# APRIL-ZJU/Ctrl-VIO

Hardware: NVIDIA H100
Metric: residual+Jacobian block evaluations per second (sliding-window LM solve) (higher is better)
Workload: dtype f64

## Files before the change

ctrl-vio_b200/csrc/chol_dag.cu:

```cuda
#include <algorithm>
#include <atomic>
#include <cstdlib>

#include "chol_tiles.cuh"
#include "dmma_tiles.cuh"
#include "kernels.h"

namespace ctvio {

namespace {

constexpr unsigned long long kSentinel = 0xFFF8C0DEC0DE0001ull;
__device__ __forceinline__ unsigned smem_u32(const void* p) { return static_cast<unsigned>(__cvta_generic_to_shared(p)); }
__device__ __forceinline__ unsigned mapa_u32(unsigned addr, unsigned rank) {
  unsigned r;
  asm volatile("mapa.shared::cluster.u32 %0, %1, %2;" : "=r"(r) : "r"(addr), "r"(rank));
  return r;
}
__device__ __forceinline__ void st_cluster2(unsigned addr, double2 v) {
  asm volatile("st.shared::cluster.v2.f64 [%0], {%1, %2};" ::"r"(addr), "d"(v.x), "d"(v.y) : "memory");
}
__device__ __forceinline__ double2 ld_shared_volatile2(const double* p) {
  double2 v;
  asm volatile("ld.volatile.shared.v2.f64 {%0, %1}, [%2];" : "=d"(v.x), "=d"(v.y) : "r"(smem_u32(p)) : "memory");
  return v;
}
__device__ __forceinline__ void cluster_arrive() { asm volatile("barrier.cluster.arrive.release.aligned;" ::: "memory"); }
__device__ __forceinline__ void cluster_wait() { asm volatile("barrier.cluster.wait.acquire.aligned;" ::: "memory"); }
__device__ __forceinline__ unsigned cluster_ctarank() {
  unsigned r;
  asm volatile("mov.u32 %0, %%cluster_ctarank;" : "=r"(r));
  return r;
}
__device__ __forceinline__ unsigned cluster_nctarank() {
  unsigned r;
  asm volatile("mov.u32 %0, %%cluster_nctarank;" : "=r"(r));
  return r;
}
__device__ __forceinline__ bool is_sentinel(double v) { return static_cast<unsigned long long>(__double_as_longlong(v)) == kSentinel; }
__device__ __forceinline__ double2 ld_relaxed2(const double* p) {
  double2 v;
  asm volatile("ld.relaxed.gpu.global.v2.f64 {%0, %1}, [%2];" : "=d"(v.x), "=d"(v.y) : "l"(p) : "memory");
  return v;
}
__device__ __forceinline__ void st_relaxed2(double* p, double2 v) {
  asm volatile("st.relaxed.gpu.global.v2.f64 [%0], {%1, %2};" ::"l"(p), "d"(v.x), "d"(v.y) : "memory");
}

__device__ __forceinline__ double ld_relaxed1(const double* p) {
  double v;
  asm volatile("ld.relaxed.gpu.global.f64 %0, [%1];" : "=d"(v) : "l"(p) : "memory");
  return v;
}
__device__ __forceinline__ void st_relaxed1(double* p, double v) {
  asm volatile("st.relaxed.gpu.global.f64 [%0], %1;" ::"l"(p), "d"(v) : "memory");
}
__device__ __forceinline__ double ld_spin(const double* p) {
  double v = ld_relaxed1(p);
  while (is_sentinel(v)) v = ld_relaxed1(p);
  return v;
}
__device__ __forceinline__ double sentinel_value() { return __longlong_as_double(static_cast<long long>(kSentinel)); }

__device__ __forceinline__ void wait_flag(const int* flag, int epoch) {
  if (threadIdx.x == 0) {
    spin_until_gpu(flag, epoch);
  }
  __syncthreads();
}
__device__ __forceinline__ void wait_flags2(const int* f1, const int* f2, int epoch) {
  if (threadIdx.x == 0) {
    spin_until_gpu(f1, epoch);
  } else if (threadIdx.x == 32) {
    spin_until_gpu(f2, epoch);
  }
  __syncthreads();
}
__device__ __forceinline__ void post_flag(int* flag, int epoch) {
  __syncthreads();
  if (threadIdx.x == 0) {
    __threadfence();
    st_release_gpu(flag, epoch);
  }
}

__device__ __forceinline__ void load_tile_cg(double* dst, const double* src, int ld, int tid) {
#pragma unroll
  for (int e = tid; e < kCholNB * kCholNB / 2; e += 256) {
    const int r = e >> 5, c = (e & 31) * 2;
    *reinterpret_cast<double2*>(dst + r * kTS + c) = __ldcg(reinterpret_cast<const double2*>(src + size_t(r) * ld + c));
  }
}
__device__ __forceinline__ void store_tile_global(double* dst, int ld, const double* src, int tid) {
#pragma unroll
  for (int e = tid; e < kCholNB * kCholNB / 2; e += 256) {
    const int r = e >> 5, c = (e & 31) * 2;
    *reinterpret_cast<double2*>(dst + size_t(r) * ld + c) = *reinterpret_cast<const double2*>(src + r * kTS + c);
  }
}
__device__ __forceinline__ double sum_partials(const double* part, int n, size_t stride, double* red, int tid) {
  const int c = tid & 63, g = tid >> 6;
  double s = 0.0;
  int q = g;
  for (; q + 12 < n; q += 16) {
    double v0 = ld_relaxed1(part + size_t(q) * stride + c), v1 = ld_relaxed1(part + size_t(q + 4) * stride + c);
    double v2 = ld_relaxed1(part + size_t(q + 8) * stride + c), v3 = ld_relaxed1(part + size_t(q + 12) * stride + c);
    while (is_sentinel(v0)) v0 = ld_relaxed1(part + size_t(q) * stride + c);
    while (is_sentinel(v1)) v1 = ld_relaxed1(part + size_t(q + 4) * stride + c);
    while (is_sentinel(v2)) v2 = ld_relaxed1(part + size_t(q + 8) * stride + c);
    while (is_sentinel(v3)) v3 = ld_relaxed1(part + size_t(q + 12) * stride + c);
    s += v0; s += v1; s += v2; s += v3;
  }
  for (; q < n; q += 4) s += ld_spin(part + size_t(q) * stride + c);
  red[g * kCholNB + c] = s;
  __syncthreads();
  return tid < kCholNB ? (red[tid] + red[kCholNB + tid]) + (red[2 * kCholNB + tid] + red[3 * kCholNB + tid]) : 0.0;
}
__device__ __forceinline__ void tile_matvec(const double* Lrm, const double* v, double* out_global, int tid,
                                            double* out_shared = nullptr) {
  const int r = tid >> 2, pt = tid & 3;
  double s = 0.0;
#pragma unroll 4
  for (int c = pt; c < kCholNB; c += 4) s = fma(Lrm[r * kTS + c], v[c], s);
  s += __shfl_xor_sync(0xffffffffu, s, 1);
  s += __shfl_xor_sync(0xffffffffu, s, 2);
  if (pt == 0) {
    st_relaxed1(out_global + r, s);
    if (out_shared) out_shared[r] = s;
  }
}
}

template <unsigned MASK>
__device__ __forceinline__ void mma_masked(Frag& f, const double* pa, int sa, const double* pb, int sb, const Lane& L, int nk4) {
#pragma unroll 4
  for (int kk = 0; kk < nk4; ++kk) {
    double av[2], bv[4];
#pragma unroll
    for (int mt = 0; mt < 2; ++mt)
      if (MASK & (0xFu << (4 * mt))) av[mt] = -pa[4 * kk * sa + 8 * L.rt[mt]];
#pragma unroll
    for (int nt = 0; nt < 4; ++nt)
      if (MASK & (0x11u << nt)) bv[nt] = pb[4 * kk * sb + 8 * L.ct[nt]];
#pragma unroll
    for (int mt = 0; mt < 2; ++mt)
#pragma unroll
      for (int nt = 0; nt < 4; ++nt)
        if ((MASK >> (4 * mt + nt)) & 1u)
          asm volatile("mma.sync.aligned.m8n8k4.row.col.f64.f64.f64.f64 {%0,%1}, {%2}, {%3}, {%0,%1};"
                       : "+d"(f.c[mt][nt][0]), "+d"(f.c[mt][nt][1]) : "d"(av[mt]), "d"(bv[nt]));
  }
}
__device__ __forceinline__ void mma_dispatch(unsigned mask, Frag& f, const double* pa, int sa, const double* pb, int sb,
                                             const Lane& L, int nk4) {
  switch (mask) {
    case 0x33u: mma_masked<0x33u>(f, pa, sa, pb, sb, L, nk4); break;
    case 0xCCu: mma_masked<0xCCu>(f, pa, sa, pb, sb, L, nk4); break;
    case 0xFFu: mma_masked<0xFFu>(f, pa, sa, pb, sb, L, nk4); break;
    case 0xF1u: mma_masked<0xF1u>(f, pa, sa, pb, sb, L, nk4); break;
    case 0x73u: mma_masked<0x73u>(f, pa, sa, pb, sb, L, nk4); break;
    case 0xF0u: mma_masked<0xF0u>(f, pa, sa, pb, sb, L, nk4); break;
    default: break;
  }
}
__device__ __forceinline__ unsigned lower_mask(int warp) {
  const int wm = warp & 3, wn = warp >> 2;
  if (wn == 0) return wm == 0 ? 0xF1u : wm == 1 ? 0x73u : 0x33u;
  return wm <= 1 ? 0xF0u : wm == 2 ? 0xF1u : 0x73u;
}
__device__ __forceinline__ unsigned slab_mask(int warp, int s) {
  const int wn = warp >> 2;
  if (wn == 0) return s == 0 ? 0x33u : s == 3 ? 0xCCu : 0u;
  return s == 1 ? 0x33u : s == 2 ? 0xCCu : 0u;
}
__device__ __forceinline__ unsigned trailing_mask(int warp, int s) {
  const int wn = warp >> 2;
  if (wn == 0) return s < 3 ? 0xCCu : 0u;
  return s == 0 ? 0xFFu : s == 1 ? 0xCCu : 0u;
}

struct CholDagArgs {
  double* M;
  int npad;
  double* Lpub;
  double* Lpub_other;
  double* Spub;
  double* Spub_other;
  const double* rhs;
  double* y;
  double* yf;
  double* part;
  double* part_other;
  int* flags;
  int epoch;
  LmScalars* scal;
  const int32_t* go;
};

#ifdef CTVIO_CHOL_TIMING
__device__ unsigned long long g_dag_stamps[32 * 16];
#define DSTAMP(j, i) do { if (threadIdx.x == 0 && (j) >= 0 && (j) < 32) { unsigned long long t_; \
    asm volatile("mov.u64 %0, %%globaltimer;" : "=l"(t_)); g_dag_stamps[(j) * 16 + (i)] = t_; } } while (0)
extern "C" int ctvio_debug_fac_clk(long long* out) {
  return cudaMemcpyFromSymbol(out, g_fac_clk, sizeof(g_fac_clk)) == cudaSuccess ? 0 : -1;
}
extern "C" int ctvio_debug_dag_stamps(unsigned long long* out) {
  return cudaMemcpyFromSymbol(out, g_dag_stamps, sizeof(g_dag_stamps)) == cudaSuccess ? 0 : -1;
}
#else
#define DSTAMP(j, i)
#endif

constexpr size_t kCholDagSmem =
    (3 * size_t(kTile) + 4 * size_t(kPacket) + 16 * size_t(kTS) + 2 * size_t(kPacket) + 256 + 7 * kCholNB + 16) * sizeof(double);

__device__ __forceinline__ void tile_matvec_t(const double* St, const double* v, double* out_global, double* red, int tid,
                                              double* out_shared = nullptr) {
  const int r = tid & 63, part = tid >> 6;
  double s = 0.0;
#pragma unroll 4
  for (int c = part; c < kCholNB; c += 4) s = fma(St[c * kTS + r], v[c], s);
  red[part * kCholNB + r] = s;
  __syncthreads();
  if (tid < kCholNB) {
    const double t = (red[tid] + red[kCholNB + tid]) + (red[2 * kCholNB + tid] + red[3 * kCholNB + tid]);
    st_relaxed1(out_global + tid, t);
    if (out_shared) out_shared[tid] = t;
  }
}

__device__ __forceinline__ void trsm_pipelined(Frag& acc, const Lane& L, double* S1, double* At, double* Bp2,
                                               const double* Lpub_col, double* slab_out, const double* Ua, const double* Ub,
                                               int tid, int jstamp, const double* pk_local = nullptr, unsigned slab_remote = 0u) {
  const int warp = tid >> 5, lane = tid & 31, g = lane >> 2, q = lane & 3;
  int goff[3], soff[3];
#pragma unroll
  for (int u = 0; u < 3; ++u) {
    const int e = tid + 256 * u;
    const int r = e / 40, c = (e - r * 40) * 2;
    goff[u] = e < 640 ? r * 80 + c : -1;
    soff[u] = r * kPS + c;
  }
  const int goff3 = tid < 128 ? (tid >> 3) * 80 + 64 + (tid & 7) * 2 : -1, soff3 = (tid >> 3) * kPS + 64 + (tid & 7) * 2;
  double2 pre[3];
  auto issue = [&](int s) {
    if (pk_local) return;
    const double* src = Lpub_col + size_t(s) * kPacketG;
    if (s < 3) {
#pragma unroll
      for (int u = 0; u < 3; ++u)
        if (goff[u] >= 0) pre[u] = ld_relaxed2(src + goff[u]);
    } else if (goff3 >= 0) {
      pre[0] = ld_relaxed2(src + goff3);
    }
  };
  auto commit = [&](int s, double* Bp) {
    if (pk_local) {
      if (s < 3) {
#pragma unroll
        for (int u = 0; u < 3; ++u)
          if (goff[u] >= 0) {
            double2 v = ld_shared_volatile2(Bp + soff[u]);
            while (is_sentinel(v.x) || is_sentinel(v.y)) v = ld_shared_volatile2(Bp + soff[u]);
          }
      } else if (goff3 >= 0) {
        double2 v = ld_shared_volatile2(Bp + soff3);
        while (is_sentinel(v.x) || is_sentinel(v.y)) v = ld_shared_volatile2(Bp + soff3);
      }
      return;
    }
    const double* src = Lpub_col + size_t(s) * kPacketG;
    if (s < 3) {
#pragma unroll
      for (int u = 0; u < 3; ++u)
        if (goff[u] >= 0) {
          while (is_sentinel(pre[u].x) || is_sentinel(pre[u].y)) pre[u] = ld_relaxed2(src + goff[u]);
          *reinterpret_cast<double2*>(Bp + soff[u]) = pre[u];
        }
    } else if (goff3 >= 0) {
      while (is_sentinel(pre[0].x) || is_sentinel(pre[0].y)) pre[0] = ld_relaxed2(src + goff3);
      *reinterpret_cast<double2*>(Bp + soff3) = pre[0];
    }
  };
  issue(0);
#pragma unroll 1
  for (int s = 0; s < 4; ++s) {
    double* Bp = pk_local ? const_cast<double*>(pk_local) + s * kPacket : Bp2 + (s & 1) * kPacket;
    if (Ua) {
      if (s == 0) mma_dispatch(slab_mask(warp, 0), acc, Ua + q * kTS + g, kTS, Ub + q * kTS + g, kTS, L, kCholNB / 4);
      if (s < 3) mma_dispatch(slab_mask(warp, s + 1), acc, Ua + q * kTS + g, kTS, Ub + q * kTS + g, kTS, L, kCholNB / 4);
    }
#pragma unroll
    for (int mt = 0; mt < 2; ++mt)
#pragma unroll
      for (int nt = 0; nt < 4; ++nt) {
        const int ct = L.ct[nt];
        if ((ct >> 1) == s) {
#pragma unroll
          for (int e = 0; e < 2; ++e) At[(8 * (ct & 1) + 2 * q + e) * kTS + L.row(mt)] = acc.c[mt][nt][e];
        }
      }
    DSTAMP(16 + jstamp, 4 * s + 0);
    commit(s, Bp);
    DSTAMP(16 + jstamp, 4 * s + 1);
    if (s < 3) issue(s + 1);
    __syncthreads();
    DSTAMP(jstamp, 8 + s);
    if (s == 3) DSTAMP(jstamp, 2);
    {
      const double* pa = At + q * kTS + 8 * warp + g;
      const double* pb = Bp + q * kPS + 64 + g;
      double2 cl = make_double2(0.0, 0.0), ch = make_double2(0.0, 0.0);
#pragma unroll
      for (int kk = 0; kk < 4; ++kk) {
        const double av = pa[4 * kk * kTS];
        if (kk < 2)
          asm volatile("mma.sync.aligned.m8n8k4.row.col.f64.f64.f64.f64 {%0,%1}, {%2}, {%3}, {%0,%1};"
                       : "+d"(cl.x), "+d"(cl.y) : "d"(av), "d"(pb[4 * kk * kPS]));
        asm volatile("mma.sync.aligned.m8n8k4.row.col.f64.f64.f64.f64 {%0,%1}, {%2}, {%3}, {%0,%1};"
                     : "+d"(ch.x), "+d"(ch.y) : "d"(av), "d"(pb[4 * kk * kPS + 8]));
      }
      double* dst = S1 + (16 * s) * kTS + 8 * warp + g;
      dst[(2 * q) * kTS] = cl.x;
      dst[(2 * q + 1) * kTS] = cl.y;
      dst[(8 + 2 * q) * kTS] = ch.x;
      dst[(8 + 2 * q + 1) * kTS] = ch.y;
    }
    DSTAMP(16 + jstamp, 4 * s + 2);
    __syncthreads();
    if (slab_out) {
#pragma unroll
      for (int u = 0; u < 2; ++u) {
        const int e = tid + 256 * u, r = e >> 5, c = (e & 31) * 2;
        const double2 v = *reinterpret_cast<const double2*>(S1 + (16 * s + r) * kTS + c);
        if (slab_remote) st_cluster2(slab_remote + unsigned(((16 * s + r) * kTS + c) * sizeof(double)), v);
        st_relaxed2(slab_out + size_t(s) * 16 * 64 + r * 64 + c, v);
      }
    }
    if (s < 3)
      mma_dispatch(trailing_mask(warp, s), acc, S1 + (16 * s + q) * kTS + g, kTS, Bp + q * kPS + g, kPS, L, 4);
    DSTAMP(16 + jstamp, 4 * s + 3);
  }
}

__global__ void __launch_bounds__(256, 1) chol_dag_kernel(CholDagArgs a) {
  extern __shared__ __align__(16) unsigned char dag_smem[];
  double* D = reinterpret_cast<double*>(dag_smem);
  double* S1 = D + kTile;
  double* S2 = S1 + kTile;
  double* Pk = S2 + kTile;
  double* At = Pk + 4 * kPacket;
  double* Bp = At + 16 * kTS;
  double* L16t = Bp + 2 * kPacket;
  double* rdiag = L16t + 256;
  double* vec = rdiag + kCholNB;
  double* vec2 = vec + kCholNB;
  double* red = vec2 + kCholNB;
  double* x16 = red + 4 * kCholNB;
  __shared__ int s_bad;
  const int tid = threadIdx.x;
  const Lane L = lane_of(tid);
  const int npad = a.npad, nb = npad / kCholNB, epoch = a.epoch;
  int* tile_ready = a.flags;
  const size_t nn = size_t(nb) * nb * kCholNB;
  double* fwd_part = a.part;
  double* bwd_part = a.part + nn;
  double* xf_pub = a.part + 2 * nn;
  double* xb_pub = xf_pub + size_t(nb) * kCholNB;
  const double sv = sentinel_value();
  const bool go = !a.go || *a.go != 0;

  const int pos = blockIdx.x, nchain = 2 * nb - 1;
  const unsigned crank = cluster_ctarank(), csize = cluster_nctarank();
  const bool dsm = csize > 1;
  const bool is_diag = pos < nchain && (pos & 1) == 0;
  const bool recv_local = dsm && pos < nchain && pos > 0 && crank != 0;
  const bool send_remote = dsm && pos + 1 < nchain && crank + 1 < csize;
  if (dsm) {
    if (recv_local) {
      double* area = is_diag ? S1 : Pk;
      const int n2 = (is_diag ? kTile : 4 * kPacket) / 2;
      for (int e = tid; e < n2; e += 256) *reinterpret_cast<double2*>(area + 2 * e) = make_double2(sv, sv);
    }
    __syncthreads();
    cluster_arrive();
  }
  pdl_wait();
  pdl_launch_dependents();
  if (!go || (dsm && pos >= nb * (nb + 1) / 2)) {
    if (dsm) cluster_wait();
    return;
  }
  if (!is_diag) {
    int i, j;
    if (pos < nchain) {
      i = (pos + 1) >> 1;
      j = i - 1;
    } else {
      int t = pos - nchain;
      j = 0;
      while (t >= nb - 2 - j) { t -= nb - 2 - j; ++j; }
      i = j + 2 + t;
    }
    const bool sub = i == j + 1;
    double* slot = a.M + size_t(i) * kCholNB * npad + j * kCholNB;
    Frag acc;
    frag_load_global(acc, slot, npad, L);
    for (int k = 0; k + 1 < j; ++k) {
      wait_flags2(tile_ready + i * nb + k, tile_ready + j * nb + k, epoch);
      load_tile_cg(S1, a.M + size_t(i) * kCholNB * npad + k * kCholNB, npad, tid);
      load_tile_cg(S2, a.M + size_t(j) * kCholNB * npad + k * kCholNB, npad, tid);
      __syncthreads();
      tile_gemm_dmma<true>(S1, S2, acc, L);
      __syncthreads();
    }
    if (j >= 1) {
      const double* srcA = a.Spub + (size_t(i) * nb + (j - 1)) * 4096;
      const double* srcB = a.Spub + (size_t(j) * nb + (j - 1)) * 4096;
      const int r0 = tid >> 5, c0 = (tid & 31) * 2;
      double2 pa[2], pb[2];
      auto issue = [&](int s) {
#pragma unroll
        for (int u = 0; u < 2; ++u) {
          pa[u] = ld_relaxed2(srcA + size_t(s) * 1024 + (r0 + 8 * u) * 64 + c0);
          pb[u] = ld_relaxed2(srcB + size_t(s) * 1024 + (r0 + 8 * u) * 64 + c0);
        }
      };
      issue(0);
#pragma unroll 1
      for (int s = 0; s < 4; ++s) {
#pragma unroll
        for (int u = 0; u < 2; ++u) {
          const size_t o = size_t(s) * 1024 + (r0 + 8 * u) * 64 + c0;
          while (is_sentinel(pa[u].x) || is_sentinel(pa[u].y)) pa[u] = ld_relaxed2(srcA + o);
          while (is_sentinel(pb[u].x) || is_sentinel(pb[u].y)) pb[u] = ld_relaxed2(srcB + o);
          *reinterpret_cast<double2*>(D + (16 * s + r0 + 8 * u) * kTS + c0) = pa[u];
          *reinterpret_cast<double2*>(S2 + (16 * s + r0 + 8 * u) * kTS + c0) = pb[u];
        }
        if (s < 3) issue(s + 1);
        __syncthreads();
        mma_dispatch(0xFFu, acc, D + (16 * s + L.q) * kTS + L.g, kTS, S2 + (16 * s + L.q) * kTS + L.g, kTS, L, 4);
      }
    }
    unsigned slab_remote = 0u;
    if (dsm) {
      cluster_wait();
      if (sub && send_remote) slab_remote = mapa_u32(smem_u32(S1), crank + 1);
    }
    trsm_pipelined(acc, L, S1, At, Bp, a.Lpub + size_t(j) * 4 * kPacketG, a.Spub + (size_t(i) * nb + j) * 4096, nullptr, nullptr, tid,
                   sub ? i : -100, (sub && recv_local) ? Pk : nullptr, slab_remote);
    __syncthreads();
    store_tile_global(slot, npad, S1, tid);
    post_flag(tile_ready + i * nb + j, epoch);
    if (!sub) {
      if (tid < kCholNB) vec[tid] = ld_spin(xf_pub + j * kCholNB + tid);
      __syncthreads();
      tile_matvec_t(S1, vec, fwd_part + (size_t(i) * nb + j) * kCholNB, red, tid);
      if (tid < kCholNB) vec[tid] = ld_spin(xb_pub + i * kCholNB + tid);
      __syncthreads();
      tile_matvec(S1, vec, bwd_part + (size_t(j) * nb + i) * kCholNB, tid);
      if (tid < kCholNB) {
        a.part_other[(size_t(i) * nb + j) * kCholNB + tid] = sv;
        a.part_other[nn + (size_t(j) * nb + i) * kCholNB + tid] = sv;
      }
    }
    {
      double* o = a.Spub_other + (size_t(i) * nb + j) * 4096;
      for (int e = tid; e < 4096 / 2; e += 256) *reinterpret_cast<double2*>(o + 2 * e) = make_double2(sv, sv);
    }
    return;
  }

  const int j = pos >> 1;
  DSTAMP(j, 0);
  Frag accD;
  frag_load_global(accD, a.M + size_t(j) * kCholNB * npad + j * kCholNB, npad, L);
  for (int k = 0; k + 1 < j; ++k) {
    wait_flag(tile_ready + j * nb + k, epoch);
    load_tile_cg(S2, a.M + size_t(j) * kCholNB * npad + k * kCholNB, npad, tid);
    __syncthreads();
    mma_dispatch(lower_mask(tid >> 5), accD, S2 + L.q * kTS + L.g, kTS, S2 + L.q * kTS + L.g, kTS, L, kCholNB / 4);
    __syncthreads();
  }
  DSTAMP(j, 1);
  {
    const double sp = sum_partials(fwd_part + size_t(j) * nb * kCholNB, j >= 1 ? j - 1 : 0, kCholNB, red, tid);
    if (tid < kCholNB) vec[tid] = a.rhs[j * kCholNB + tid] - sp;
  }
  if (j >= 1) {
    const double* src = a.Spub + (size_t(j) * nb + (j - 1)) * 4096;
    const int r0 = tid >> 5, c0 = (tid & 31) * 2;
    double2 pre[2];
    auto issue = [&](int s) {
      pre[0] = ld_relaxed2(src + size_t(s) * 1024 + r0 * 64 + c0);
      pre[1] = ld_relaxed2(src + size_t(s) * 1024 + (r0 + 8) * 64 + c0);
    };
    if (!recv_local) issue(0);
#pragma unroll 1
    for (int s = 0; s < 4; ++s) {
      if (recv_local) {
#pragma unroll
        for (int u = 0; u < 2; ++u) {
          const double* w = S1 + (16 * s + r0 + 8 * u) * kTS + c0;
          double2 v = ld_shared_volatile2(w);
          while (is_sentinel(v.x) || is_sentinel(v.y)) v = ld_shared_volatile2(w);
        }
      } else {
#pragma unroll
        for (int u = 0; u < 2; ++u) {
          const double* w = src + size_t(s) * 1024 + (r0 + 8 * u) * 64 + c0;
          while (is_sentinel(pre[u].x) || is_sentinel(pre[u].y)) pre[u] = ld_relaxed2(w);
          *reinterpret_cast<double2*>(S1 + (16 * s + r0 + 8 * u) * kTS + c0) = pre[u];
        }
        if (s < 3) issue(s + 1);
      }
      __syncthreads();
      DSTAMP(j, 8 + s);
      if (s == 3) DSTAMP(j, 2);
      mma_dispatch(lower_mask(tid >> 5), accD, S1 + (16 * s + L.q) * kTS + L.g, kTS, S1 + (16 * s + L.q) * kTS + L.g, kTS, L, 4);
    }
    DSTAMP(j, 3);
  }
  frag_store(D, accD, L);
  __syncthreads();
  DSTAMP(j, 4);
  double* own = red;
  double* gpk = a.Lpub + size_t(j) * 4 * kPacketG;
  unsigned rpk = 0u;
  if (send_remote) rpk = mapa_u32(smem_u32(Pk), crank + 1);
  auto side = [&](int step) {
    if (j == 0) return;
    const int tt = tid - 32;
    if (step == 1 && tt < kCholNB) {
      vec2[tt] = ld_spin(xf_pub + (j - 1) * kCholNB + tt);
    } else if (step == 2 && tt < 128) {
      const int r = tt >> 1, pt = tt & 1;
      double acc = 0.0;
#pragma unroll 8
      for (int c = pt; c < kCholNB; c += 2) acc = fma(S1[c * kTS + r], vec2[c], acc);
      acc += __shfl_xor_sync(0xffffffffu, acc, 1);
      if (pt == 0) own[r] = acc;
    }
  };
  auto pub = [&](int s) {
    if (dsm && s == 0) cluster_wait();
    const int tt = tid - 32;
    const double* src = Pk + s * kPacket;
    double* dst = gpk + size_t(s) * kPacketG;
    for (int e = tt; e < 16 * 40; e += 224) {
      const int r = e / 40, c = (e - r * 40) * 2;
      double2 v = *reinterpret_cast<const double2*>(src + r * kPS + c);
      if (c < 16 * (s + 1) && c < 64) v = make_double2(0.0, 0.0);
      if (rpk) st_cluster2(rpk + unsigned((s * kPacket + r * kPS + c) * sizeof(double)), v);
      st_relaxed2(dst + r * 80 + c, v);
    }
  };
  auto pub_last = [&]() {
    if (dsm && tid < 32) cluster_wait();
    if (tid < 128) {
      const int r = tid >> 3, c = 64 + (tid & 7) * 2;
      const double2 v = *reinterpret_cast<const double2*>(Pk + 3 * kPacket + r * kPS + c);
      if (rpk) st_cluster2(rpk + unsigned((3 * kPacket + r * kPS + c) * sizeof(double)), v);
      st_relaxed2(gpk + size_t(3) * kPacketG + r * 80 + c, v);
    }
  };
  if (!factor_64_pipe(D, Pk, L16t, rdiag, &s_bad, pub, pub_last, side) && tid == 0) a.scal->chol_fail = 1;
  DSTAMP(j, 5);
  if (j >= 1 && tid < kCholNB) vec[tid] -= own[tid];
  __syncthreads();
  block_solve_packets<true>(Pk, vec, x16, tid);
  if (tid < kCholNB) {
    st_relaxed1(xf_pub + j * kCholNB + tid, vec[tid]);
    a.yf[j * kCholNB + tid] = vec[tid];
    vec2[tid] = vec[tid];
  }
  DSTAMP(j, 6);
  if (j == nb - 1) {
    __syncthreads();
    block_solve_packets<false>(Pk, vec, x16, tid);
    if (tid < kCholNB) {
      st_relaxed1(xb_pub + j * kCholNB + tid, vec[tid]);
      vec2[tid] = vec[tid];
    }
  } else {
    inverse_from_packets(Pk, D, tid);
    {
      const double sp = sum_partials(bwd_part + (size_t(j) * nb + j + 1) * kCholNB, nb - 1 - j, kCholNB, red, tid);
      if (tid < kCholNB) vec[tid] = vec2[tid] - sp;
    }
    __syncthreads();
    tile_matvec_t(D, vec, xb_pub + j * kCholNB, red, tid, vec2);
  }
  __syncthreads();
  if (j >= 1) {
    tile_matvec(S1, vec2, bwd_part + (size_t(j - 1) * nb + j) * kCholNB, tid);
  }
  if (tid < kCholNB) a.y[j * kCholNB + tid] = vec2[tid];
  DSTAMP(j, 7);
  {
    double* o = a.Lpub_other + size_t(j) * 4 * kPacketG;
    for (int e = tid; e < 4 * kPacketG / 2; e += 256) *reinterpret_cast<double2*>(o + 2 * e) = make_double2(sv, sv);
    if (tid < kCholNB) {
      a.part_other[2 * nn + size_t(j) * kCholNB + tid] = sv;
      a.part_other[2 * nn + size_t(nb + j) * kCholNB + tid] = sv;
      if (j >= 1) a.part_other[nn + (size_t(j - 1) * nb + j) * kCholNB + tid] = sv;
    }
  }
}

constexpr int kDagCluster = 8;
static std::atomic<long long> g_dag_cluster_launches{0};
static std::atomic<long long> g_dag_plain_launches{0};
static int dag_grid(int nb) { return nb * (nb + 1) / 2; }

bool chol_dag_supported(int npad, int n_sm) { return dag_grid(npad / kCholNB) <= n_sm; }

static size_t dag_part_half(int npad) {
  const size_t nb = npad / kCholNB;
  return (2 * nb * nb + 2 * nb) * kCholNB;
}
size_t chol_dag_part_len(int npad) { return 2 * dag_part_half(npad); }
size_t chol_dag_flags_len(int npad) {
  const size_t nb = npad / kCholNB;
  return nb * nb;
}
static size_t dag_pub_len(int npad) {
  const size_t nb = npad / kCholNB;
  return nb * 4 * kPacketG + nb * nb * 4096;
}
size_t chol_dag_lpub_len(int npad) { return size_t(npad) * kCholNB + 2 * dag_pub_len(npad); }

__global__ void fill_sentinel_kernel(double* p, size_t n) {
  const size_t i = size_t(blockIdx.x) * blockDim.x + threadIdx.x;
  if (i < n) p[i] = __longlong_as_double(static_cast<long long>(kSentinel));
}
int launch_chol_dag_init(double* linv_buf, double* part_buf, int npad, cudaStream_t s) {
  const size_t n = 2 * dag_pub_len(npad), m = chol_dag_part_len(npad);
  fill_sentinel_kernel<<<unsigned((n + 255) / 256), 256, 0, s>>>(linv_buf + size_t(npad) * kCholNB, n);
  fill_sentinel_kernel<<<unsigned((m + 255) / 256), 256, 0, s>>>(part_buf, m);
  return 2;
}

int launch_chol_dag(const LinearLaunch& l, cudaStream_t s, bool* tile_dag) {
  static PerDeviceOnce once;
  static std::atomic<unsigned> epoch_src{0};
  if (once.first()) cudaFuncSetAttribute(chol_dag_kernel, cudaFuncAttributeMaxDynamicSharedMemorySize, int(kCholDagSmem));
  CholDagArgs a;
  const size_t half = size_t(l.npad / kCholNB) * 4 * kPacketG;
  const unsigned parity = l.chol_seq ? ((*l.chol_seq)++ & 1u) : 0u;
  a.M = l.M; a.npad = l.npad;
  const size_t shalf = size_t(l.npad / kCholNB) * size_t(l.npad / kCholNB) * 4096;
  double* pk = l.Linv + size_t(l.npad) * kCholNB;
  a.Lpub = pk + parity * half;
  a.Lpub_other = pk + (parity ^ 1u) * half;
  a.Spub = pk + 2 * half + parity * shalf;
  a.Spub_other = pk + 2 * half + (parity ^ 1u) * shalf;
  a.part = l.chol_part + parity * dag_part_half(l.npad);
  a.part_other = l.chol_part + (parity ^ 1u) * dag_part_half(l.npad);
  a.rhs = l.rhs; a.y = l.y; a.yf = l.yf;
  a.flags = l.chol_flags; a.scal = l.scal; a.go = l.go;
  a.epoch = int(epoch_src.fetch_add(1, std::memory_order_relaxed) % 0x7ffffffeu) + 1;
  static std::atomic<int> cluster_state{-1};
  bool want_cluster = cluster_state.load(std::memory_order_relaxed) != 0;
  if (const char* v = std::getenv("CTVIO_CHOL_CLUSTER"))
    if (v[0] == '0') want_cluster = false;
  if (std::getenv("NV_COMPUTE_PROFILER_PERFWORKS_DIR") || std::getenv("NV_NSIGHT_INJECTION_TRANSPORT_TYPE") ||
      std::getenv("CUDA_INJECTION64_PATH") || std::getenv("NSYS_PROFILING_SESSION_ID"))
    want_cluster = false;
  const int total = dag_grid(l.npad / kCholNB);
  if (want_cluster) {
    cudaLaunchConfig_t cfg = {};
    cfg.gridDim = dim3(unsigned((total + kDagCluster - 1) / kDagCluster * kDagCluster));
    cfg.blockDim = dim3(256);
    cfg.dynamicSmemBytes = kCholDagSmem;
    cfg.stream = s;
    cudaLaunchAttribute at[3];
    at[0].id = cudaLaunchAttributeClusterDimension;
    at[0].val.clusterDim.x = kDagCluster; at[0].val.clusterDim.y = 1; at[0].val.clusterDim.z = 1;
    at[1].id = cudaLaunchAttributeCooperative;
    at[1].val.cooperative = 1;
    at[2].id = cudaLaunchAttributeProgrammaticStreamSerialization;
    at[2].val.programmaticStreamSerializationAllowed = 1;
    cfg.attrs = at;
    cfg.numAttrs = l.pdl ? 3 : 2;
    cudaError_t cerr = cudaLaunchKernelEx(&cfg, chol_dag_kernel, a);
    if (cerr != cudaSuccess && l.pdl) {
      cudaGetLastError();
      cfg.numAttrs = 2;
      cerr = cudaLaunchKernelEx(&cfg, chol_dag_kernel, a);
    }
    if (cerr == cudaSuccess) {
      cluster_state.store(1, std::memory_order_relaxed);
      g_dag_cluster_launches.fetch_add(1, std::memory_order_relaxed);
      if (tile_dag) *tile_dag = true;
      return 1;
    }
    cudaGetLastError();
    if (cluster_state.load(std::memory_order_relaxed) < 0) cluster_state.store(0, std::memory_order_relaxed);
  }
  void* args[] = {&a};
  const cudaError_t err = cudaLaunchCooperativeKernel(reinterpret_cast<void*>(chol_dag_kernel), dim3(total),
                                                      dim3(256), args, kCholDagSmem, s);
  if (err != cudaSuccess) {
    cudaGetLastError();
    if (tile_dag) *tile_dag = false;
    return launch_chol_coop(l, s);
  }
  g_dag_plain_launches.fetch_add(1, std::memory_order_relaxed);
  if (tile_dag) *tile_dag = true;
  return 1;
}

const double* chol_dag_last_packets(const double* linv_buf, int npad, unsigned chol_seq) {
  const size_t half = size_t(npad / kCholNB) * 4 * kPacketG;
  return linv_buf + size_t(npad) * kCholNB + ((chol_seq - 1u) & 1u) * half;
}

extern "C" long long ctvio_debug_chol_cluster_launches() { return g_dag_cluster_launches.load(); }
extern "C" long long ctvio_debug_chol_plain_launches() { return g_dag_plain_launches.load(); }

}
```

Measured before the change: 36.78 million.

## Send backward-solve partial via cluster DSMEM and hoist sentinel resets before PDL wait

The diagonal block now pushes its backward-substitution partial sum straight into the shared memory of the diagonal block two ranks earlier in the cluster, instead of going through global memory. The receiving block spins on a local volatile shared load. The sentinel resets of the other ping-pong buffers move from the end of each block to before pdl_wait, so they overlap the previous launch and no longer sit on the critical tail. Risks: a cluster peer might exit while a remote store is still pending, and the receiving block only picks up the local partial when recv_bwd holds.

```diff
diff --git a/ctrl-vio_b200/csrc/chol_dag.cu b/ctrl-vio_b200/csrc/chol_dag.cu
--- a/ctrl-vio_b200/csrc/chol_dag.cu
+++ b/ctrl-vio_b200/csrc/chol_dag.cu
@@ -20,6 +20,14 @@
 __device__ __forceinline__ void st_cluster2(unsigned addr, double2 v) {
   asm volatile("st.shared::cluster.v2.f64 [%0], {%1, %2};" ::"r"(addr), "d"(v.x), "d"(v.y) : "memory");
 }
+__device__ __forceinline__ void st_cluster1(unsigned addr, double v) {
+  asm volatile("st.shared::cluster.f64 [%0], %1;" ::"r"(addr), "d"(v) : "memory");
+}
+__device__ __forceinline__ double ld_shared_volatile1(const double* p) {
+  double v;
+  asm volatile("ld.volatile.shared.f64 %0, [%1];" : "=d"(v) : "r"(smem_u32(p)) : "memory");
+  return v;
+}
 __device__ __forceinline__ double2 ld_shared_volatile2(const double* p) {
   double2 v;
   asm volatile("ld.volatile.shared.v2.f64 {%0, %1}, [%2];" : "=d"(v.x), "=d"(v.y) : "r"(smem_u32(p)) : "memory");
@@ -98,10 +106,17 @@
     *reinterpret_cast<double2*>(dst + size_t(r) * ld + c) = *reinterpret_cast<const double2*>(src + r * kTS + c);
   }
 }
-__device__ __forceinline__ double sum_partials(const double* part, int n, size_t stride, double* red, int tid) {
+__device__ __forceinline__ double sum_partials(const double* part, int n, size_t stride, double* red, int tid,
+                                               const double* first_local = nullptr) {
   const int c = tid & 63, g = tid >> 6;
   double s = 0.0;
   int q = g;
+  if (first_local && g == 0 && n > 0) {
+    double v = ld_shared_volatile1(first_local + c);
+    while (is_sentinel(v)) v = ld_shared_volatile1(first_local + c);
+    s += v;
+    q = 4;
+  }
   for (; q + 12 < n; q += 16) {
     double v0 = ld_relaxed1(part + size_t(q) * stride + c), v1 = ld_relaxed1(part + size_t(q + 4) * stride + c);
     double v2 = ld_relaxed1(part + size_t(q + 8) * stride + c), v3 = ld_relaxed1(part + size_t(q + 12) * stride + c);
@@ -117,7 +132,7 @@
   return tid < kCholNB ? (red[tid] + red[kCholNB + tid]) + (red[2 * kCholNB + tid] + red[3 * kCholNB + tid]) : 0.0;
 }
 __device__ __forceinline__ void tile_matvec(const double* Lrm, const double* v, double* out_global, int tid,
-                                            double* out_shared = nullptr) {
+                                            unsigned out_remote = 0u) {
   const int r = tid >> 2, pt = tid & 3;
   double s = 0.0;
 #pragma unroll 4
@@ -125,8 +140,8 @@
   s += __shfl_xor_sync(0xffffffffu, s, 1);
   s += __shfl_xor_sync(0xffffffffu, s, 2);
   if (pt == 0) {
-    st_relaxed1(out_global + r, s);
-    if (out_shared) out_shared[r] = s;
+    if (out_remote) st_cluster1(out_remote + unsigned(r * sizeof(double)), s);
+    else st_relaxed1(out_global + r, s);
   }
 }
 }
@@ -199,20 +214,27 @@
 
 #ifdef CTVIO_CHOL_TIMING
 __device__ unsigned long long g_dag_stamps[32 * 16];
+__device__ unsigned long long g_dag_exit[256];
 #define DSTAMP(j, i) do { if (threadIdx.x == 0 && (j) >= 0 && (j) < 32) { unsigned long long t_; \
     asm volatile("mov.u64 %0, %%globaltimer;" : "=l"(t_)); g_dag_stamps[(j) * 16 + (i)] = t_; } } while (0)
+#define DEXIT() do { if (threadIdx.x == 0 && blockIdx.x < 256) { unsigned long long t_; \
+    asm volatile("mov.u64 %0, %%globaltimer;" : "=l"(t_)); g_dag_exit[blockIdx.x] = t_; } } while (0)
 extern "C" int ctvio_debug_fac_clk(long long* out) {
   return cudaMemcpyFromSymbol(out, g_fac_clk, sizeof(g_fac_clk)) == cudaSuccess ? 0 : -1;
 }
 extern "C" int ctvio_debug_dag_stamps(unsigned long long* out) {
   return cudaMemcpyFromSymbol(out, g_dag_stamps, sizeof(g_dag_stamps)) == cudaSuccess ? 0 : -1;
 }
+extern "C" int ctvio_debug_dag_exit(unsigned long long* out) {
+  return cudaMemcpyFromSymbol(out, g_dag_exit, sizeof(g_dag_exit)) == cudaSuccess ? 0 : -1;
+}
 #else
 #define DSTAMP(j, i)
+#define DEXIT()
 #endif
 
 constexpr size_t kCholDagSmem =
-    (3 * size_t(kTile) + 4 * size_t(kPacket) + 16 * size_t(kTS) + 2 * size_t(kPacket) + 256 + 7 * kCholNB + 16) * sizeof(double);
+    (3 * size_t(kTile) + 4 * size_t(kPacket) + 16 * size_t(kTS) + 2 * size_t(kPacket) + 256 + 8 * kCholNB + 16) * sizeof(double);
 
 __device__ __forceinline__ void tile_matvec_t(const double* St, const double* v, double* out_global, double* red, int tid,
                                               double* out_shared = nullptr) {
@@ -357,6 +379,7 @@
   double* vec2 = vec + kCholNB;
   double* red = vec2 + kCholNB;
   double* x16 = red + 4 * kCholNB;
+  double* bwd_in = x16 + 16;
   __shared__ int s_bad;
   const int tid = threadIdx.x;
   const Lane L = lane_of(tid);
@@ -376,23 +399,11 @@
   const bool is_diag = pos < nchain && (pos & 1) == 0;
   const bool recv_local = dsm && pos < nchain && pos > 0 && crank != 0;
   const bool send_remote = dsm && pos + 1 < nchain && crank + 1 < csize;
-  if (dsm) {
-    if (recv_local) {
-      double* area = is_diag ? S1 : Pk;
-      const int n2 = (is_diag ? kTile : 4 * kPacket) / 2;
-      for (int e = tid; e < n2; e += 256) *reinterpret_cast<double2*>(area + 2 * e) = make_double2(sv, sv);
-    }
-    __syncthreads();
-    cluster_arrive();
-  }
-  pdl_wait();
-  pdl_launch_dependents();
-  if (!go || (dsm && pos >= nb * (nb + 1) / 2)) {
-    if (dsm) cluster_wait();
-    return;
-  }
-  if (!is_diag) {
-    int i, j;
+  const bool recv_bwd = dsm && is_diag && pos + 2 < nchain && crank + 2 < csize;
+  const bool send_bwd = dsm && is_diag && pos >= 2 && crank >= 2;
+  const bool real = pos < nb * (nb + 1) / 2;
+  int i = 0, j = pos >> 1;
+  if (!is_diag && real) {
     if (pos < nchain) {
       i = (pos + 1) >> 1;
       j = i - 1;
@@ -402,6 +413,42 @@
       while (t >= nb - 2 - j) { t -= nb - 2 - j; ++j; }
       i = j + 2 + t;
     }
+  }
+  if (dsm) {
+    if (recv_local) {
+      double* area = is_diag ? S1 : Pk;
+      const int n2 = (is_diag ? kTile : 4 * kPacket) / 2;
+      for (int e = tid; e < n2; e += 256) *reinterpret_cast<double2*>(area + 2 * e) = make_double2(sv, sv);
+    }
+    if (recv_bwd && tid < kCholNB) bwd_in[tid] = sv;
+    __syncthreads();
+    cluster_arrive();
+  }
+  if (go && real) {
+    if (is_diag) {
+      double* o = a.Lpub_other + size_t(j) * 4 * kPacketG;
+      for (int e = tid; e < 4 * kPacketG / 2; e += 256) *reinterpret_cast<double2*>(o + 2 * e) = make_double2(sv, sv);
+      if (tid < kCholNB) {
+        a.part_other[2 * nn + size_t(j) * kCholNB + tid] = sv;
+        a.part_other[2 * nn + size_t(nb + j) * kCholNB + tid] = sv;
+        if (j >= 1) a.part_other[nn + (size_t(j - 1) * nb + j) * kCholNB + tid] = sv;
+      }
+    } else {
+      if (i != j + 1 && tid < kCholNB) {
+        a.part_other[(size_t(i) * nb + j) * kCholNB + tid] = sv;
+        a.part_other[nn + (size_t(j) * nb + i) * kCholNB + tid] = sv;
+      }
+      double* o = a.Spub_other + (size_t(i) * nb + j) * 4096;
+      for (int e = tid; e < 4096 / 2; e += 256) *reinterpret_cast<double2*>(o + 2 * e) = make_double2(sv, sv);
+    }
+  }
+  pdl_wait();
+  pdl_launch_dependents();
+  if (!go || !real) {
+    if (dsm) cluster_wait();
+    return;
+  }
+  if (!is_diag) {
     const bool sub = i == j + 1;
     double* slot = a.M + size_t(i) * kCholNB * npad + j * kCholNB;
     Frag acc;
@@ -459,19 +506,11 @@
       if (tid < kCholNB) vec[tid] = ld_spin(xb_pub + i * kCholNB + tid);
       __syncthreads();
       tile_matvec(S1, vec, bwd_part + (size_t(j) * nb + i) * kCholNB, tid);
-      if (tid < kCholNB) {
-        a.part_other[(size_t(i) * nb + j) * kCholNB + tid] = sv;
-        a.part_other[nn + (size_t(j) * nb + i) * kCholNB + tid] = sv;
-      }
-    }
-    {
-      double* o = a.Spub_other + (size_t(i) * nb + j) * 4096;
-      for (int e = tid; e < 4096 / 2; e += 256) *reinterpret_cast<double2*>(o + 2 * e) = make_double2(sv, sv);
-    }
+    }
+    DEXIT();
     return;
   }
 
-  const int j = pos >> 1;
   DSTAMP(j, 0);
   Frag accD;
   frag_load_global(accD, a.M + size_t(j) * kCholNB * npad + j * kCholNB, npad, L);
@@ -585,27 +624,22 @@
   } else {
     inverse_from_packets(Pk, D, tid);
     {
-      const double sp = sum_partials(bwd_part + (size_t(j) * nb + j + 1) * kCholNB, nb - 1 - j, kCholNB, red, tid);
+      const double sp = sum_partials(bwd_part + (size_t(j) * nb + j + 1) * kCholNB, nb - 1 - j, kCholNB, red, tid,
+                                     recv_bwd ? bwd_in : nullptr);
       if (tid < kCholNB) vec[tid] = vec2[tid] - sp;
     }
     __syncthreads();
     tile_matvec_t(D, vec, xb_pub + j * kCholNB, red, tid, vec2);
   }
+  DSTAMP(j, 12);
   __syncthreads();
   if (j >= 1) {
-    tile_matvec(S1, vec2, bwd_part + (size_t(j - 1) * nb + j) * kCholNB, tid);
+    tile_matvec(S1, vec2, bwd_part + (size_t(j - 1) * nb + j) * kCholNB, tid,
+                send_bwd ? mapa_u32(smem_u32(bwd_in), crank - 2) : 0u);
   }
   if (tid < kCholNB) a.y[j * kCholNB + tid] = vec2[tid];
   DSTAMP(j, 7);
-  {
-    double* o = a.Lpub_other + size_t(j) * 4 * kPacketG;
-    for (int e = tid; e < 4 * kPacketG / 2; e += 256) *reinterpret_cast<double2*>(o + 2 * e) = make_double2(sv, sv);
-    if (tid < kCholNB) {
-      a.part_other[2 * nn + size_t(j) * kCholNB + tid] = sv;
-      a.part_other[2 * nn + size_t(nb + j) * kCholNB + tid] = sv;
-      if (j >= 1) a.part_other[nn + (size_t(j - 1) * nb + j) * kCholNB + tid] = sv;
-    }
-  }
+  DEXIT();
 }
 
 constexpr int kDagCluster = 8;
```

Measured after the change: 37.01 million, median of 6. About the same (+0.6%).
